# floe/backscrub

Hardware: AMD Instinct MI355X
Metric: composited frames/sec at 640×480 (batch), 1/2/4/8 MI355X + mask IoU vs CPU ref (higher is better)
Workload: dtype f32 (network) / u8 (image kernels)

## Files before the change

### backscrub_amd/csrc/bsx_api.hip

```cpp
#include "debug_switches.hpp"
#include <hip/hip_runtime.h>

#include <cmath>
#include <cstdarg>
#include <cstdio>
#include <cstdlib>
#include <cstring>
#include <map>
#include <memory>
#include <string>
#include <vector>

#include "../../include/bsx.h"
#include "gen_mid.hpp"
#include "gen_seg.hpp"
#include "kernels.hpp"
#include "roctx_ranges.hpp"
#include "rtc.hpp"
#include "plan.hpp"
#include "tflite_model.hpp"

using namespace bsx;

namespace {
// ... 191 lines not shown
  return "";
}

int model_type_from_name(const std::string& n) {
  if (n.find("body-pix") != n.npos) return BSX_MODEL_BODYPIX;
  if (n.find("deeplab") != n.npos) return BSX_MODEL_DEEPLAB;
  if (n.find("segm_") != n.npos) return BSX_MODEL_MEET;
  if (n.find("selfie") != n.npos) return BSX_MODEL_MLKIT;
  return BSX_MODEL_UNKNOWN;
}

int init_device_state(bsx_ctx* c) {
  BSX_HIP(c, hipStreamCreateWithFlags(&c->own_stream, hipStreamNonBlocking));
  const size_t N = (size_t)c->n_streams;
  BSX_HIP(c, hipMalloc(&c->d_arena, c->plan.arena_floats_per_stream * N * sizeof(float)));
  BSX_HIP(c, hipMalloc(&c->d_net_in, N * c->inW * c->inH * c->inC * sizeof(float)));
  BSX_HIP(c, hipMalloc(&c->d_net_in_u8, N * c->inW * c->inH * sizeof(uint32_t)));
  BSX_HIP(c, hipMalloc(&c->d_net_out, N * c->outW * c->outH * c->outC * sizeof(float)));
  BSX_HIP(c, hipMalloc(&c->d_weights, std::max<size_t>(c->plan.weights.size(), 4) * sizeof(float)));
  BSX_HIP(c, hipMemcpy(c->d_weights, c->plan.weights.data(), c->plan.weights.size() * sizeof(float), hipMemcpyHostToDevice));
  BSX_HIP(c, hipMalloc(&c->d_weights16, std::max<size_t>(c->plan.weights16.size(), 8) * sizeof(uint16_t)));
  BSX_HIP(c, hipMemcpy(c->d_weights16, c->plan.weights16.data(), c->plan.weights16.size() * sizeof(uint16_t), hipMemcpyHostToDevice));
  if (const char* m = getenv("BSX_F16_GEMM")) c->f16_terms = !strcmp(m, "off") ? 0 : (!strcmp(m, "fast") ? 1 : (!strcmp(m, "fast16") ? 17 : 3));
  c->use_program = !c->plan.program.empty() && BSX_DBG_ENV("BSX_NO_FRAME_PROGRAM") == nullptr &&
                   (c->plan.seg.on || c->plan.program_lds_tensors >= c->plan.program_global_tensors || BSX_DBG_ENV("BSX_FORCE_FRAME_PROGRAM") != nullptr);
  if (c->use_program) {
    BSX_HIP(c, hipMalloc(&c->d_program, c->plan.program.size() * sizeof(MicroOp)));
    BSX_HIP(c, hipMemcpy(c->d_program, c->plan.program.data(), c->plan.program.size() * sizeof(MicroOp), hipMemcpyHostToDevice));
    BSX_HIP(c, frame_program_prepare(c->plan.program_lds_floats));
    if (c->plan.seg.on) BSX_HIP(c, seg_prepare());
// ... 154 lines not shown
  if (logits || !c->seg_fn[2]) return launch_seg_tail(sp.tail, c->d_arena, pf, c->d_net_out, ofinal, c->d_weights, logits, n, s, c->act16);
  SegTail d = sp.tail; float* arena = c->d_arena; float* no = c->d_net_out; const float* w = c->d_weights; int nf = n;
  void* args[] = {&d, &arena, &pf, &no, &ofinal, &w, &nf};
  return seg_launch(c->seg_fn[2], d.tiles_y * d.tiles_x, n, d.lds_floats, s, args);
}

int run_infer(bsx_ctx* c, int n, hipStream_t s, bool logits = true, int slot = 0) {
  bsx_roctx::Range range("bsx:network");
  if (c->use_program && c->plan.seg.on) {
    const SegPlan& sp = c->plan.seg;
    const long pf = (long)c->plan.arena_floats_per_stream;
    BSX_HIP(c, seg_head(c, n, s));
    BSX_HIP(c, seg_k2(c, n, s));
    BSX_HIP(c, launch_program(c, n, s));
    BSX_HIP(c, seg_k3(c, n, s));
    if (sp.tail.pre_gate_off >= 0) BSX_HIP(c, launch_seg_gate(sp.tail.gate, c->d_arena, pf, c->d_weights, sp.tail.pre_gate_off, n, s));
    if (!logits) { const int frc = state_write_fence(c, s); if (frc) return frc; }
    BSX_HIP(c, seg_tail(c, c->d_ofinal + (size_t)slot * c->outW * c->outH, logits, n, s));
    return BSX_OK;
  }
  if (c->use_program) {
    BSX_HIP(c, launch_program(c, n, s));
    return BSX_OK;
  }
  const bool fused_tail = !logits && argmax_tail(c);
  const size_t ns = c->plan.steps.size() - (fused_tail ? 1 : 0);
  for (size_t i = 0; i < ns; i++)
    BSX_HIP(c, launch_step(c->plan.steps[i], c->plan, c->d_arena, c->d_net_in, c->d_net_out, c->d_weights, n, c->n_streams, s, c->d_weights16, c->f16_terms, c->in_u8 ? c->d_net_in_u8 : nullptr, c->norm_scale, c->norm_offset));
  if (fused_tail) {
    const Step& last = c->plan.steps.back();
    { const int frc = state_write_fence(c, s); if (frc) return frc; }
// ... 505 lines not shown
      if (!d_frames || !prep_yuyv_fusable(c->width, c->roi, c->tab_down.tab)) return BSX_EINVAL;
      return run_prep(c, d_frames, n, s, true, true);
    default: return BSX_EINVAL;
  }
}

int bsx_profile_batch(bsx_ctx* c, const uint8_t* d_frames, const uint8_t* d_bg, size_t bg_stride, uint8_t* d_out, int n, int iters,
                      bsx_launch_stat* out, int cap, void* stream) {
  if (!c || !d_frames || !d_bg || !d_out || !out || n <= 0 || n > c->n_streams || iters <= 0) return BSX_EINVAL;
  if (c->pend.active) { c->last_error = "error: a pipelined composite is pending (flush with bsx_step_batch_pipelined(ctx, NULL, ...) first)\n"; return BSX_EINVAL; }
  DeviceGuard guard(c->device);
  hipStream_t s = pick(c, stream);
  const bool seg = c->use_program && c->plan.seg.on;
  const bool fused_decode = infer_decodes(c);
  const bool atail = argmax_tail(c);
  const int n_net = c->use_program ? (seg ? (c->plan.seg.tail.pre_gate_off >= 0 ? 6 : 5) : 1) : (int)c->plan.steps.size();
  const bool fuse_tail = !c->onmask && !c->no_mask_blend_fusion &&
                         mask_blend_fusable(c->width, c->height, c->roi, d_bg, bg_stride, d_frames, d_out);
  const int L = 1 + n_net + (fused_decode ? 0 : 1) + (fuse_tail ? 1 : 2) + (fuse_tail ? 1 : 0);
  if (cap < L) return BSX_EINVAL;
  std::vector<hipEvent_t> ev((size_t)L + 1);
  for (auto& e : ev) BSX_HIP(c, hipEventCreate(&e));
  std::vector<double> sum(L, 0.0);
  const double N = n, px = (double)c->width * c->height;
  for (int it = 0; it < iters; it++) {
    int k = 0;
    BSX_HIP(c, hipEventRecord(ev[0], s));
#define BSX_TIMED(call)                                    \
    do {                                                   \
      BSX_HIP(c, (call));                                  \
      BSX_HIP(c, hipEventRecord(ev[k + 1], s));            \
      k++;                                                 \
    } while (0)
    BSX_TIMED(launch_prep_fused(d_frames, c->width, c->height, c->roi, c->in_u8 ? nullptr : c->tensor_ptr(c->plan.input), c->in_u8 ? c->d_net_in_u8 : nullptr, c->inW, c->inH, c->in_roi,
                                c->tab_down.tab, c->bilateral, n, s));
    const long pf = (long)c->plan.arena_floats_per_stream;
    if (seg) {
      const SegPlan& sp = c->plan.seg;
      BSX_TIMED(seg_head(c, n, s));
      BSX_TIMED(seg_k2(c, n, s));
      BSX_TIMED(launch_program(c, n, s));
      BSX_TIMED(seg_k3(c, n, s));
      if (sp.tail.pre_gate_off >= 0) BSX_TIMED(launch_seg_gate(sp.tail.gate, c->d_arena, pf, c->d_weights, sp.tail.pre_gate_off, n, s));
      BSX_TIMED(seg_tail(c, c->d_ofinal, !fused_decode, n, s));
    } else if (c->use_program)
      BSX_TIMED(launch_program(c, n, s));
    else {
      for (size_t si = 0; si + (atail ? 1 : 0) < c->plan.steps.size(); si++)
        BSX_TIMED(launch_step(c->plan.steps[si], c->plan, c->d_arena, c->d_net_in, c->d_net_out, c->d_weights, n, c->n_streams, s, c->d_weights16, c->f16_terms, c->in_u8 ? c->d_net_in_u8 : nullptr, c->norm_scale, c->norm_offset));
      if (atail) BSX_TIMED(launch_resize_argmax_iir(c->plan.steps.back(), c->d_arena + (size_t)c->plan.tensor_off[c->plan.steps.back().in0] * (size_t)c->n_streams,
                                                    c->d_ofinal, n, s, c->tail_generic));
    }
    if (!fused_decode) BSX_TIMED(launch_decode(c->model_type, c->tensor_ptr(c->plan.output), c->d_ofinal, c->outW * c->outH, c->outC, n, s));
    if (fuse_tail) {
      BSX_TIMED(launch_mask_blend(c->d_ofinal, c->outW, c->outH, c->in_roi, c->tab_up.tab, c->d_masks, c->width, c->height, c->roi, d_bg, bg_stride,
                                  d_frames, d_out, n, s));
      BSX_TIMED(launch_blend(d_bg, bg_stride, d_frames, c->d_masks, d_out, (size_t)c->width * c->height, n, s));
    } else {
// ... 13 lines not shown
  int j = 0;
  const double canvas = (double)c->inW * c->inH;
  const double touched = (double)std::min(c->roi.w, 2 * c->in_roi.w) * (double)std::min(c->roi.h, 2 * c->in_roi.h);
  put(j++, "prep", N * (3.0 * touched + (c->in_u8 ? 4.0 : 12.0) * canvas), 0);
  if (seg) {
    const std::vector<Step>& S = c->plan.steps;
    const int NS = (int)S.size();
    auto macs = [&](int a, int b) { double m = 0; for (int i = a; i <= b; i++) m += S[i].macs; return m; };
    const SegPlan& sp = c->plan.seg;
    const double eA = 16.0 * sp.head.H1 * sp.head.W1, eb0 = 16.0 * sp.head.H2 * sp.head.W2, ec0 = (double)sp.k2.dw.C * sp.k2.H3 * sp.k2.W3;
    const double elo2 = 16.0 * sp.k3.HL * sp.k3.WL, elo = 16.0 * sp.k3.H2 * sp.k3.W2;
    const double ein = (double)c->inW * c->inH * c->inC, eout = (double)c->outW * c->outH * c->outC;
    put(j++, "seg_head", N * ((c->in_u8 ? 4.0 * c->inW * c->inH : 4.0 * ein) + 4.0 * (eA + eb0)), N * 2.0 * macs(0, 2));
    put(j++, "seg_k2", N * 4.0 * (eb0 + eb0 + ec0), N * 2.0 * macs(3, 8));
    put(j++, "frame_program", N * 4.0 * (ec0 + elo2) + 4.0 * c->plan.weights.size(), N * 2.0 * macs(9, NS - 11));
    put(j++, "seg_k3", N * 4.0 * (eb0 + elo2 + elo), N * 2.0 * macs(NS - 10, NS - 8));
    if (sp.tail.pre_gate_off >= 0) put(j++, "seg_gate", N * 4.0 * (16.0 * (sp.tail.gate.part[0].n + sp.tail.gate.part[1].n) + 16.0), 0);
    put(j++, fused_decode ? "seg_tail+decode" : "seg_tail", N * (4.0 * (eA + elo) + (fused_decode ? 2.0 * c->outW * c->outH : 4.0 * eout)), N * 2.0 * macs(NS - 7, NS - 1));
  } else if (c->use_program) {
    double io = (double)c->inW * c->inH * c->inC + (double)c->outW * c->outH * c->outC;
    put(j++, "frame_program", N * io * 4.0 + 4.0 * c->plan.weights.size(), N * 2.0 * c->plan.macs_per_frame);
  } else
  for (const Step& st : c->plan.steps) {
    double in = (double)st.H * st.W * st.Cin, o = (double)st.OH * st.OW * st.Cout, b = 0;
    switch (st.kind) {
      case StepKind::Eltwise: b = in + o + (st.elt == kEltUnary ? 0 : (st.bcast1 ? st.Cin : in)) + (st.elt == kEltMulAdd ? in : 0); break;
      case StepKind::Concat: b = 2 * o; break;
      case StepKind::Gap: b = in + st.Cin; break;
      default: b = in + o + (st.residual >= 0 ? o : 0) + (st.in_scale >= 0 ? st.Cin : 0); break;
    }
    const bool is_tail = atail && &st == &c->plan.steps.back();
    const bool ir_on = c->d_weights16 && c->f16_terms > 0;
// ... 194 lines not shown
```

### backscrub_amd/csrc/gen_seg.cpp

```cpp
#include "gen_seg.hpp"

#include <cstdarg>
#include <cstdio>

namespace bsx {
namespace {

const char kSegSource[] =
#include "seg_rtc_src.inc"
    ;

}

std::string seg_constants_text(const SegPlan& sp, const char* pre) {
  std::string out;
  auto P = [&](const char* fmt, ...) {
    char buf[1024];
    va_list ap;
    va_start(ap, fmt);
    vsnprintf(buf, sizeof buf, fmt, ap);
    va_end(ap);
    out += buf;
  };
  auto conv = [&](const char* n, const SegConvW& c) { P("  t.%s.w_off = %lldll; t.%s.b_off = %lldll; t.%s.Cin = %d; t.%s.Cout = %d; t.%s.cout_pad = %d; t.%s.act = %d;\n", n, c.w_off, n, c.b_off, n, c.Cin, n, c.Cout, n, c.cout_pad, n, c.act); };
// ... 5 lines not shown
      P("  t.%s.fc[%d].w_off = %lldll; t.%s.fc[%d].b_off = %lldll; t.%s.fc[%d].Cin = %d; t.%s.fc[%d].Cout = %d; t.%s.fc[%d].act = %d;\n", n, i, g_.fc[i].w_off, n, i, g_.fc[i].b_off, n, i, g_.fc[i].Cin, n, i,
              g_.fc[i].Cout, n, i, g_.fc[i].act);
    }
  };
  const SegHead& H = sp.head; const SegK2& K2 = sp.k2; const SegK3& K3 = sp.k3; const SegTail& T = sp.tail;
  P("// segment descriptors of the loaded graph as constants (gen_seg.cpp: seg_constants_text)\nconstexpr SegHead %sHEAD = [] { SegHead t{};\n", pre);
  P("  t.H0 = %d; t.W0 = %d; t.H1 = %d; t.W1 = %d; t.H2 = %d; t.W2 = %d; t.stem_pt = %d; t.stem_pl = %d; t.dw_pt = %d; t.dw_pl = %d;\n", H.H0, H.W0, H.H1, H.W1, H.H2, H.W2, H.stem_pt, H.stem_pl, H.dw_pt, H.dw_pl);
  conv("stem", H.stem); conv("pw", H.pw); dw("dw", H.dw);
  P("  t.a_off = %lldll; t.b0_off = %lldll; t.part_a_off = %lldll; t.part_b0_off = %lldll; t.TR = %d; t.TC = %d; t.tiles_y = %d; t.tiles_x = %d; t.lds_floats = %d; t.rw = %d; t.m_ct = %uu;\n  return t; }();\n",
          H.a_off, H.b0_off, H.part_a_off, H.part_b0_off, H.TR, H.TC, H.tiles_y, H.tiles_x, H.lds_floats, H.rw, H.m_ct);
  P("constexpr SegK2 %sK2 = [] { SegK2 t{};\n  t.H2 = %d; t.W2 = %d; t.H3 = %d; t.W3 = %d; t.dw_pt = %d; t.dw_pl = %d;\n", pre, K2.H2, K2.W2, K2.H3, K2.W3, K2.dw_pt, K2.dw_pl);
  gate("gate", K2.gate); conv("pw_a", K2.pw_a); conv("pw_b", K2.pw_b); dw("dw", K2.dw);
  P("  t.b0_off = %lldll; t.B_off = %lldll; t.c0_off = %lldll; t.part_B_off = %lldll; t.TR = %d; t.TC = %d; t.tiles_y = %d; t.tiles_x = %d; t.lds_floats = %d; t.rw = %d; t.m_ct = %uu;\n  return t; }();\n",
          K2.b0_off, K2.B_off, K2.c0_off, K2.part_B_off, K2.TR, K2.TC, K2.tiles_y, K2.tiles_x, K2.lds_floats, K2.rw, K2.m_ct);
  P("constexpr SegK3 %sK3 = [] { SegK3 t{};\n  t.H2 = %d; t.W2 = %d; t.HL = %d; t.WL = %d; t.half_pixel = %d; t.align_corners = %d;\n", pre, K3.H2, K3.W2, K3.HL, K3.WL, K3.half_pixel, K3.align_corners);
  conv("pw1", K3.pw1); conv("pw2", K3.pw2); dw("dw", K3.dw);
  P("  t.skip_off = %lldll; t.lo2_off = %lldll; t.g_off = %lldll; t.lo_off = %lldll; t.part_lo_off = %lldll; t.TR = %d; t.TC = %d; t.tiles_y = %d; t.tiles_x = %d; t.lds_floats = %d; t.lo_floats = %d; t.hs = (float)%.9g; t.ws = (float)%.9g;\n  return t; }();\n",
          K3.skip_off, K3.lo2_off, K3.g_off, K3.lo_off, K3.part_lo_off, K3.TR, K3.TC, K3.tiles_y, K3.tiles_x, K3.lds_floats, K3.lo_floats, (double)K3.hs, (double)K3.ws);
  P("constexpr SegTail %sTAIL = [] { SegTail t{};\n  t.H1 = %d; t.W1 = %d; t.HL = %d; t.WL = %d; t.H0 = %d; t.W0 = %d; t.half_pixel = %d; t.align_corners = %d;\n", pre, T.H1, T.W1, T.HL, T.WL, T.H0, T.W0, T.half_pixel, T.align_corners);
  gate("gate", T.gate); conv("pw", T.pw); dw("dw", T.dw);
  P("  t.tc_w_off = %lldll; t.tc_b_off = %lldll; t.Co = %d; t.act3 = %d; t.model_type = %d; t.skip_off = %lldll; t.lo_off = %lldll; t.pre_gate_off = %lldll; t.TR = %d; t.TC = %d; t.tiles_y = %d; t.tiles_x = %d; "
             "t.lds_floats = %d; t.lo_floats = %d; t.hs = (float)%.9g; t.ws = (float)%.9g;\n  return t; }();\n",
          T.tc_w_off, T.tc_b_off, T.Co, T.act3, T.model_type, T.skip_off, T.lo_off, T.pre_gate_off, T.TR, T.TC, T.tiles_y, T.tiles_x, T.lds_floats, T.lo_floats, (double)T.hs, (double)T.ws);
  return out;
}

std::string generate_seg_source(const Plan& plan, bool h16, bool u8in, std::string* why) {
  auto fail = [&](const char* m) { if (why) *why = m; return std::string(); };
  if (!plan.seg.on) return fail("no segment kernels in this plan");
  const SegPlan& sp = plan.seg;
  const bool sig = sp.tail.act3 == kActSigmoid;
// ... 14 lines not shown
```

### backscrub_amd/csrc/kernels_seg.hip

```cpp
#ifndef __HIPCC_RTC__
#include <hip/hip_runtime.h>
#endif
#ifndef BSX_SEG_RTC
#include "debug_switches.hpp"

#include <algorithm>
#include <cstdlib>

#include "kernels.hpp"
#include "mfma_tile.hpp"
#include "segments.hpp"
#endif

#if defined(BSX_SEG_RTC)
#define BSX_SEG_D(T, NAME) constexpr T d = kSeg##NAME; (void)d_rt
#elif defined(BSX_SEG_PROBE)
#define BSX_SEG_D(T, NAME) constexpr T d = kProbe##NAME; (void)d_rt
#else
#define BSX_SEG_D(T, NAME) const T& d = d_rt
#endif

namespace bsx {
#ifdef BSX_SEG_RTC
namespace segrtc {
BSX_SEG_CONSTANTS
constexpr bool STEM_HSWISH = BSX_SEG_HS != 0, H16 = BSX_SEG_H16 != 0, U8IN = BSX_SEG_U8 != 0, LOGITS = false, SIGMOID = BSX_SEG_SIG != 0;
constexpr int CO = BSX_SEG_CO;
#else
namespace {
#endif
#ifdef BSX_SEG_PROBE
#include BSX_SEG_PROBE
#endif

extern __shared__ __attribute__((aligned(16))) float seg_smem[];

constexpr int kScrGate = 0;
constexpr int kScrRed = 96;
constexpr int kScrFloats = kSegScratchFloats;

__device__ __forceinline__ float4 ld4(const float* p) { return *reinterpret_cast<const float4*>(p); }
__device__ __forceinline__ void st4(float* p, float4 v) { *reinterpret_cast<float4*>(p) = v; }
// ... 42 lines not shown
__device__ __forceinline__ float4 acc_quad(const f4acc acc) { return make_float4(acc[0], acc[1], acc[2], acc[3]); }
__device__ __forceinline__ f4acc mma16(const float4 a, const float (&wr)[4]) {
  f4acc acc = {0.f, 0.f, 0.f, 0.f};
  acc = __builtin_amdgcn_mfma_f32_16x16x4f32(wr[0], a.x, acc, 0, 0, 0);
  acc = __builtin_amdgcn_mfma_f32_16x16x4f32(wr[1], a.y, acc, 0, 0, 0);
  acc = __builtin_amdgcn_mfma_f32_16x16x4f32(wr[2], a.z, acc, 0, 0, 0);
  acc = __builtin_amdgcn_mfma_f32_16x16x4f32(wr[3], a.w, acc, 0, 0, 0);
  return acc;
}
__device__ __forceinline__ void load_wtile(float (&wr)[4], const float* __restrict__ w, const SegConvW& c, int n0, int li, int g) {
#pragma unroll
  for (int r = 0; r < 4; r++) wr[r] = (w + c.w_off)[(unsigned)((4 * g + r) * c.cout_pad + n0 + li)];
}

constexpr int kGateStageFloats = kSegGateStageFloats;
__device__ __forceinline__ void seg_gate(const SegGate& gt, const float* __restrict__ fa, const float* __restrict__ w, float* scr, float* stage) {
  float* s_gate = scr + kScrGate;
  if (gt.timing_skip) { if (threadIdx.x < 16) s_gate[threadIdx.x] = 0.5f; __syncthreads(); return; }
  float* s_mean = scr + kScrGate + 16;
  float* s_hid = scr + kScrGate + 48;
  const int tid = threadIdx.x;
  const SegFc &f1 = gt.fc[0], &f2 = gt.fc[1];
  const int w1n = f1.Cin * f1.Cout, w2n = gt.n_fc == 2 ? f2.Cin * f2.Cout : 0;
  float* ps = stage;
  float* w1 = ps + 512;
  float* b1 = w1 + w1n;
  float* w2 = b1 + f1.Cout;
  float* b2 = w2 + w2n;
  {
    const int c = tid & 15, slice = tid >> 4;
    for (int k = 0; k < gt.n_parts; k++) {
      const float* src = fa + gt.part[k].off;
      float s = 0.f;
#pragma unroll 4
      for (int i = slice; i < gt.part[k].n; i += 16) s += src[(unsigned)(i * 16 + c)];
      ps[k * 256 + slice * 16 + c] = s;
    }
  }
  {
    const float* g1 = w + f1.w_off;
    const float* g2 = w + f2.w_off;
    for (int i = tid; i < w1n; i += kSegThreads) w1[i] = g1[(unsigned)i];
    for (int i = tid; i < w2n; i += kSegThreads) w2[i] = g2[(unsigned)i];
    if (tid < f1.Cout) b1[tid] = (w + f1.b_off)[(unsigned)tid];
    if (gt.n_fc == 2 && tid < f2.Cout) b2[tid] = (w + f2.b_off)[(unsigned)tid];
  }
  __syncthreads();
  const int Cm = gt.sum_parts ? 16 : 16 * gt.n_parts;
  if (tid < Cm) {
    float m = 0.f;
// ... 32 lines not shown
template <int MODE>
__device__ __forceinline__ void wave_reduce16(float4 v, float* s_red, int wave, int lane) {
  if (MODE == 0) {
    v.x += dpp_row_shr<1>(v.x); v.y += dpp_row_shr<1>(v.y); v.z += dpp_row_shr<1>(v.z); v.w += dpp_row_shr<1>(v.w);
    v.x += dpp_row_shr<2>(v.x); v.y += dpp_row_shr<2>(v.y); v.z += dpp_row_shr<2>(v.z); v.w += dpp_row_shr<2>(v.w);
    v.x += dpp_row_shr<4>(v.x); v.y += dpp_row_shr<4>(v.y); v.z += dpp_row_shr<4>(v.z); v.w += dpp_row_shr<4>(v.w);
    v.x += dpp_row_shr<8>(v.x); v.y += dpp_row_shr<8>(v.y); v.z += dpp_row_shr<8>(v.z); v.w += dpp_row_shr<8>(v.w);
    const int li = lane & 15;
    if (li >= 12) st4(s_red + (wave * 4 + (15 - li)) * 16 + 4 * (lane >> 4), li == 15 ? v : f4zero());
  } else {
    v.x += dpp_row_shr<4>(v.x); v.y += dpp_row_shr<4>(v.y); v.z += dpp_row_shr<4>(v.z); v.w += dpp_row_shr<4>(v.w);
    v.x += dpp_row_shr<8>(v.x); v.y += dpp_row_shr<8>(v.y); v.z += dpp_row_shr<8>(v.z); v.w += dpp_row_shr<8>(v.w);
    if ((lane & 12) == 12) st4(s_red + (wave * 4 + (lane >> 4)) * 16 + 4 * (lane & 3), v);
  }
}
__device__ __forceinline__ void store_partials(const float* s_red, float* dst ) {
  if (threadIdx.x < 16) {
    float s = 0.f;
#pragma unroll
    for (int j = 0; j < 16; j++) s += s_red[j * 16 + threadIdx.x];
    dst[threadIdx.x] = s;
  }
}

__device__ __forceinline__ void up_axis(int o, float scale, bool half_pixel, int in_size, int* lo, int* hi, float* frac) {
  const float v = half_pixel ? __fadd_rn(__fmul_rn((float)o + 0.5f, scale), -0.5f) : __fmul_rn((float)o, scale);
  const float fl = floorf(v);
  *lo = max((int)fl, 0);
  *hi = min((int)ceilf(v), in_size - 1);
  *frac = v - (float)*lo;
}
__device__ __forceinline__ float up_scale(int in, int out, bool align) { return (align && out > 1) ? (float)(in - 1) / (float)(out - 1) : (float)in / (float)out; }

__device__ __forceinline__ float quad_reduce_scatter(float p0, float p1, float p2, float p3, int quad) {
  const bool b0 = quad & 1, b1 = quad & 2;
  const float klo = (b0 ? p1 : p0) + dpp_quad(b0 ? p0 : p1, 1);
// ... 357 lines not shown
    float4 a;
    a.x = fmaf(sk.x, gv.x, fmaf(td.x, w11, fmaf(tc.x, w01, fmaf(tb.x, w10, ta.x * w00))));
    a.y = fmaf(sk.y, gv.y, fmaf(td.y, w11, fmaf(tc.y, w01, fmaf(tb.y, w10, ta.y * w00))));
    a.z = fmaf(sk.z, gv.z, fmaf(td.z, w11, fmaf(tc.z, w01, fmaf(tb.z, w10, ta.z * w00))));
    a.w = fmaf(sk.w, gv.w, fmaf(td.w, w11, fmaf(tc.w, w01, fmaf(tb.w, w10, ta.w * w00))));
    const f4acc acc = mma16(a, wr);
    float4 v = acc_quad(acc);
    v = (ecol_in && row_in) ? clamp4(f4add(v, bias), cl) : f4zero();
    if (xe < ZC) st4(z_t + zy * 256 + col_a(xe, g), v);
  }
}

#ifdef BSX_SEG_RTC
extern "C" __global__ __launch_bounds__(kSegThreads) void bsx_seg_k3(
#else
template <bool H16>
__global__ __launch_bounds__(kSegThreads) void seg_k3_k(
#endif
    const SegK3 d_rt, float* __restrict__ arena, long per_frame, const float* __restrict__ w, int n_frames) {
  BSX_SEG_D(SegK3, K3);
  unsigned f_, t_;
  xcd_frame_tile((unsigned)(d.tiles_y * d.tiles_x), (unsigned)n_frames, &f_, &t_);
  const int f = (int)f_, ty = (int)t_ / d.tiles_x, tx = (int)t_ - ty * d.tiles_x;
  const int r0 = ty * d.TR, c0 = tx * d.TC, ZH = d.TR + 2, ZC = d.TC + 2;
  float* fa = arena + (size_t)f * (size_t)per_frame;
  float* z_t = seg_smem + kScrFloats;
  float* l_t = z_t + ZH * 256;
  float* lo_out = fa + d.lo_off;
  const int tid = threadIdx.x, lane = tid & 63, wave = wave_uniform(tid >> 6), li = lane & 15, g = lane >> 4, cq4 = 4 * g;
  const GatedPre pre = gated_prefetch<H16>(fa + d.skip_off, fa + d.lo2_off, d.H2, d.W2, d.HL, d.WL, d.half_pixel != 0, d.hs, d.ws, r0, c0, ZH, ZC, l_t);
  if (tid < 16) seg_smem[kScrGate + tid] = fa[d.g_off + tid];
// ... 14 lines not shown
  const int xe = li;
  for (int py = wave; py < d.TR && r0 + py < d.H2; py += 4) {
    const f4v zc = ldv(z_t + (py + 1) * 256 + coz[1]);
    const float4 dv = clamp4(tof4(dw3x3(z_t, 256, py, coz, wd) + bias_d), cl_dw);
    const f4acc acc = mma16(f4add(dv, tof4(zc)), wr);
    float4 v = acc_quad(acc);
    if (xe < d.TC && c0 + xe < d.W2) {
      v = clamp4(f4add(v, bias2), cl_2);
      stg4<H16>(lo_out, (unsigned)(((r0 + py) * d.W2 + c0 + xe) * 16 + cq4), v);
      sum = f4add(sum, v);
    }
  }
  float* s_red = seg_smem + kScrRed;
  wave_reduce16<0>(sum, s_red, wave, lane);
  __syncthreads();
  store_partials(s_red, fa + d.part_lo_off + (long)t_ * 16);
}

#ifdef BSX_SEG_RTC
extern "C" __global__ __launch_bounds__(kSegThreads) __attribute__((amdgpu_waves_per_eu(5, 5))) void bsx_seg_tail(
#else
template <int CO, bool LOGITS, bool SIGMOID, bool H16>
__global__ __launch_bounds__(kSegThreads) __attribute__((amdgpu_waves_per_eu(5, 5))) void seg_tail_k(
#endif
    const SegTail d_rt, float* __restrict__ arena, long per_frame, float* __restrict__ net_out,
                                                          uint8_t* __restrict__ ofinal, const float* __restrict__ w, int n_frames) {
  BSX_SEG_D(SegTail, TAIL);
  unsigned f_, t_;
  xcd_frame_tile((unsigned)(d.tiles_y * d.tiles_x), (unsigned)n_frames, &f_, &t_);
  const int f = (int)f_, ty = (int)t_ / d.tiles_x, tx = (int)t_ - ty * d.tiles_x;
  const int r0 = ty * d.TR, c0 = tx * d.TC, ZH = d.TR + 2, ZC = d.TC + 2;
// ... 75 lines not shown
template <class K>
hipError_t allow_lds(K kernel, int lds_bytes) {
  return hipFuncSetAttribute(reinterpret_cast<const void*>(kernel), hipFuncAttributeMaxDynamicSharedMemorySize, lds_bytes);
}
#endif

}

#ifndef BSX_SEG_RTC
hipError_t seg_prepare() {
  const int full = 160 * 1024;
  hipError_t e = hipSuccess;
  auto one = [&](auto k) { if (e == hipSuccess) e = allow_lds(k, full); };
  one(seg_head_k<true, false, false>); one(seg_head_k<false, false, false>); one(seg_head_k<true, true, false>); one(seg_head_k<false, true, false>);
  one(seg_head_k<true, false, true>); one(seg_head_k<false, false, true>); one(seg_head_k<true, true, true>); one(seg_head_k<false, true, true>);
  one(seg_k2_k<false>); one(seg_k2_k<true>); one(seg_k3_k<false>); one(seg_k3_k<true>);
  one(seg_tail_k<1, false, true, false>); one(seg_tail_k<1, true, true, false>); one(seg_tail_k<1, false, false, false>); one(seg_tail_k<1, true, false, false>);
  one(seg_tail_k<2, false, false, false>); one(seg_tail_k<2, true, false, false>);
  one(seg_tail_k<1, false, true, true>); one(seg_tail_k<1, true, true, true>); one(seg_tail_k<1, false, false, true>); one(seg_tail_k<1, true, false, true>);
  one(seg_tail_k<2, false, false, true>); one(seg_tail_k<2, true, false, true>);
  return e;
}

static int xcd_frames(int n) { static const bool on = !(BSX_DBG_ENV("BSX_XCD_TILES") && atoi(BSX_DBG_ENV("BSX_XCD_TILES")) == 0); return on ? n : 0; }

hipError_t launch_seg_head(const SegHead& d, float* arena, long per_frame, const void* net_in, const float* weights, int n, hipStream_t s, bool h16, bool u8, float in_scale,
                           float in_offset) {
  const dim3 grid((unsigned)(d.tiles_y * d.tiles_x) * (unsigned)n);
  const size_t lds = (size_t)d.lds_floats * sizeof(float);
  const bool hs = d.stem.act == kActHswish;
  const float* in = static_cast<const float*>(net_in);
  if (u8 && 2 * (2 * d.TC + 1) + 1 > 64) return hipErrorInvalidValue;
#define BSX_HEAD(HS, H, U) seg_head_k<HS, H, U><<<grid, kSegThreads, lds, s>>>(d, arena, per_frame, in, weights, in_scale, in_offset, xcd_frames(n))
  if (hs) { if (h16) { if (u8) BSX_HEAD(true, true, true); else BSX_HEAD(true, true, false); } else { if (u8) BSX_HEAD(true, false, true); else BSX_HEAD(true, false, false); } }
  else { if (h16) { if (u8) BSX_HEAD(false, true, true); else BSX_HEAD(false, true, false); } else { if (u8) BSX_HEAD(false, false, true); else BSX_HEAD(false, false, false); } }
#undef BSX_HEAD
  return hipGetLastError();
}
hipError_t launch_seg_k2(const SegK2& d, float* arena, long per_frame, const float* weights, int n, hipStream_t s, bool h16) {
  const dim3 grid((unsigned)(d.tiles_y * d.tiles_x) * (unsigned)n);
  if (h16) seg_k2_k<true><<<grid, kSegThreads, (size_t)d.lds_floats * sizeof(float), s>>>(d, arena, per_frame, weights, xcd_frames(n));
  else seg_k2_k<false><<<grid, kSegThreads, (size_t)d.lds_floats * sizeof(float), s>>>(d, arena, per_frame, weights, xcd_frames(n));
  return hipGetLastError();
}
hipError_t launch_seg_k3(const SegK3& d, float* arena, long per_frame, const float* weights, int n, hipStream_t s, bool h16) {
  const dim3 grid((unsigned)(d.tiles_y * d.tiles_x) * (unsigned)n);
  if (h16) seg_k3_k<true><<<grid, kSegThreads, (size_t)d.lds_floats * sizeof(float), s>>>(d, arena, per_frame, weights, xcd_frames(n));
  else seg_k3_k<false><<<grid, kSegThreads, (size_t)d.lds_floats * sizeof(float), s>>>(d, arena, per_frame, weights, xcd_frames(n));
  return hipGetLastError();
}
template <bool H16>
static hipError_t launch_seg_tail_t(const SegTail& d, float* arena, long per_frame, float* net_out, uint8_t* ofinal, const float* weights, bool logits, int n, hipStream_t s) {
  const dim3 grid((unsigned)(d.tiles_y * d.tiles_x) * (unsigned)n);
  static const int wgs_cap = BSX_DBG_ENV("BSX_SEG_TAIL_WGS") ? atoi(BSX_DBG_ENV("BSX_SEG_TAIL_WGS")) : 0;
  size_t lds = (size_t)d.lds_floats * sizeof(float);
  if (wgs_cap > 0) lds = std::max(lds, (size_t)(160 * 1024 / (wgs_cap + 1) + 256));
  const bool sig = d.act3 == kActSigmoid;
  if (d.Co == 2 && !sig) {
    if (logits) seg_tail_k<2, true, false, H16><<<grid, kSegThreads, lds, s>>>(d, arena, per_frame, net_out, ofinal, weights, xcd_frames(n));
    else seg_tail_k<2, false, false, H16><<<grid, kSegThreads, lds, s>>>(d, arena, per_frame, net_out, ofinal, weights, xcd_frames(n));
  } else if (d.Co == 1 && sig) {
    if (logits) seg_tail_k<1, true, true, H16><<<grid, kSegThreads, lds, s>>>(d, arena, per_frame, net_out, ofinal, weights, xcd_frames(n));
    else seg_tail_k<1, false, true, H16><<<grid, kSegThreads, lds, s>>>(d, arena, per_frame, net_out, ofinal, weights, xcd_frames(n));
// ... 20 lines not shown
```

### backscrub_amd/csrc/plan.cpp

```cpp
#include "debug_switches.hpp"
#include "plan.hpp"
#include "gen_seg.hpp"
#include "gen_mid.hpp"

#include <algorithm>
#include <cmath>
#include <cstdio>
#include <cstdlib>
#include <cstring>
#include <map>

namespace bsx {
namespace {

void conv_geometry(int in, int k, int s, int d, bool same, int* out, int* pad) {
  int eff = (k - 1) * d + 1;
  *out = same ? (in + s - 1) / s : (in + s - eff) / s;
  int total = (*out - 1) * s + eff - in;
  *pad = total > 0 ? total / 2 : 0;
}

uint16_t f32_to_f16_rn(float f) {
  uint32_t x; memcpy(&x, &f, 4);
  const uint32_t sign = (x >> 16) & 0x8000u;
// ... 600 lines not shown
  tl.pw = conv_w(tpw); tl.dw = dw_w(tdw); tl.tc_w_off = (long long)ttc.w_off; tl.tc_b_off = (long long)ttc.b_off; tl.Co = ttc.Cout; tl.act3 = ttc.act;
  split(tl.H1, tgt[6], &tl.TR, &tl.tiles_y); split(tl.W1, tgt[7], &tl.TC, &tl.tiles_x);
  tl.hs = seg_up_scale(tl.HL, tl.H1, tl.align_corners != 0); tl.ws = seg_up_scale(tl.WL, tl.W1, tl.align_corners != 0);
  if (!BSX_DBG_ENV("BSX_SEG_LO_WORST")) tl.lo_floats = seg_lo_window_floats(tl.H1, tl.W1, tl.HL, tl.WL, tl.half_pixel != 0, tl.align_corners != 0, tl.TR, tl.TC, tl.tiles_y, tl.tiles_x);
  tl.lds_floats = seg_tail_lds_floats(tl);
  if (tl.TC > 14 || tl.TR > 18) return seg_fail(33);
  const int lds_cap = 160 * 256;
  if (h.lds_floats > lds_cap || k2.lds_floats > lds_cap || k3.lds_floats > lds_cap || tl.lds_floats > lds_cap) return seg_fail(24);
  if (ttc.OH != 2 * tpw.OH || ttc.OW != 2 * tpw.OW || h.H2 != k3.H2 || h.W2 != k3.W2) return seg_fail(25);
  if (h.tiles_y * h.tiles_x > 1024 || k2.tiles_y * k2.tiles_x > 1024 || k3.tiles_y * k3.tiles_x > 1024) return seg_fail(26);

  const int pA = synth("partials(A)", h.tiles_y * h.tiles_x, 16), pb0 = synth("partials(b0)", h.tiles_y * h.tiles_x, 16);
  const int pB = synth("partials(B)", k2.tiles_y * k2.tiles_x, 16), plo = synth("partials(lo)", k3.tiles_y * k3.tiles_x, 16);
  const int pgt = BSX_DBG_ENV("BSX_SEG_NO_GATE_KERNEL") ? -1 : synth("gate(tail)", 1, 16);
  if (pgt >= 0) plan->tensor_off[pgt] = reserve(16);
  for (int t : {A, b0, B, c0, lo2, lo, kf2.out, pA, pb0, pB, plo}) plan->tensor_off[t] = reserve(g.tensors[t].elems());
  for (int t : {hpw.out, g1.out, f1a.out, f1b.out, pwb.out, up2, kg.out, kf1.out, kp1.out, kd.out, up, tg.out, tf1.out, tf2.out, tpw.out, tdw.out})
    if (t != g.output) plan->tensor_off[t] = -1;
  plan->arena_floats_per_stream = top;

  h.a_off = plan->tensor_off[A]; h.b0_off = plan->tensor_off[b0]; h.part_a_off = plan->tensor_off[pA]; h.part_b0_off = plan->tensor_off[pb0];
  k2.b0_off = plan->tensor_off[b0]; k2.B_off = plan->tensor_off[B]; k2.c0_off = plan->tensor_off[c0]; k2.part_B_off = plan->tensor_off[pB];
  k2.gate.n_parts = 1; k2.gate.n_fc = 2; k2.gate.sum_parts = 0;
  k2.gate.part[0].off = plan->tensor_off[pb0]; k2.gate.part[0].n = h.tiles_y * h.tiles_x; k2.gate.part[0].C = 16; k2.gate.part[0].hw = (float)(h.H2 * h.W2);
  k2.gate.fc[0] = fc_w(f1a); k2.gate.fc[1] = fc_w(f1b);
  k3.skip_off = plan->tensor_off[B]; k3.lo2_off = plan->tensor_off[lo2]; k3.g_off = plan->tensor_off[kf2.out]; k3.lo_off = plan->tensor_off[lo];
  k3.part_lo_off = plan->tensor_off[plo];
  tl.skip_off = plan->tensor_off[A]; tl.lo_off = plan->tensor_off[lo];
  tl.gate.n_parts = 2; tl.gate.n_fc = 2; tl.gate.sum_parts = tg.gap_sum ? 1 : 0;
  tl.gate.part[0].off = plan->tensor_off[pA]; tl.gate.part[0].n = h.tiles_y * h.tiles_x; tl.gate.part[0].C = 16; tl.gate.part[0].hw = (float)(h.H1 * h.W1);
  tl.gate.part[1].off = plan->tensor_off[plo]; tl.gate.part[1].n = k3.tiles_y * k3.tiles_x; tl.gate.part[1].C = 16; tl.gate.part[1].hw = (float)(k3.H2 * k3.W2);
  tl.gate.fc[0] = fc_w(tf1); tl.gate.fc[1] = fc_w(tf2);
  if (BSX_DBG_ENV("BSX_SEG_GATE_SKIP")) k2.gate.timing_skip = tl.gate.timing_skip = 1;
  if (const char* e = BSX_DBG_ENV("BSX_SEG_SKIP")) sscanf(e, "%d,%d,%d,%d", &h.dbg_skip, &k2.dbg_skip, &k3.dbg_skip, &tl.dbg_skip);
  tl.pre_gate_off = pgt >= 0 ? plan->tensor_off[pgt] : -1;
  if (tl.gate.fc[0].Cin != (tl.gate.sum_parts ? 16 : 32) || k2.gate.fc[0].Cin != 16) return seg_fail(27);

  std::vector<Step> mid(S.begin() + 9, S.begin() + (NS - 14));
  Step gate = kg;
  gate.concat_in = {B, lo2};
  gate.in0 = B;
  gate.label += "*";
  mid.push_back(gate); mid.push_back(kf1); mid.push_back(kf2);
  std::map<int, int> part_n, part_hw;
  part_n[B] = k2.tiles_y * k2.tiles_x; part_hw[B] = k2.H2 * k2.W2;
  const long B_real = plan->tensor_off[B];
  plan->tensor_off[B] = plan->tensor_off[pB];
  build_frame_program(g, plan, mid, {c0, B, lo2, kf2.out}, part_n, part_hw);
  plan->tensor_off[B] = B_real;
  if (plan->program.empty()) return seg_fail(28);
// ... 558 lines not shown
```

### backscrub_amd/csrc/segments.hpp

```cpp
#pragma once
#ifndef BSX_SEG_RTC
#include <algorithm>
#include <cmath>
#include <cstdint>
#endif

namespace bsx {

struct SegConvW { long long w_off = 0, b_off = 0; int Cin = 0, Cout = 0, cout_pad = 0, act = 0; };
struct SegDwW { long long w_off = 0, b_off = 0; int C = 0, act = 0; };
struct SegFc { long long w_off = 0, b_off = 0; int Cin = 0, Cout = 0, act = 0; };
struct SegPart { long long off = 0; int n = 0, C = 0; float hw = 1.f; };
struct SegGate {
  int n_parts = 0, sum_parts = 0, n_fc = 0;
  int timing_skip = 0;
  SegPart part[2];
  SegFc fc[2];
};

constexpr int kSegThreads = 256;
constexpr int kSegMaxC = 16;

struct SegHead {
  int H0 = 0, W0 = 0, H1 = 0, W1 = 0, H2 = 0, W2 = 0;
// ... 21 lines not shown
  int rw = 0;
  unsigned m_ct = 0;
};

struct SegK3 {
  int H2 = 0, W2 = 0, HL = 0, WL = 0;
  int half_pixel = 0, align_corners = 0;
  SegConvW pw1, pw2;
  SegDwW dw;
  long long skip_off = 0, lo2_off = 0, g_off = 0, lo_off = 0, part_lo_off = 0;
  int TR = 0, TC = 0, tiles_y = 0, tiles_x = 0;
  int lds_floats = 0;
  int lo_floats = 0;
  float hs = 0.f, ws = 0.f;
  int dbg_skip = 0;
};

struct SegTail {
  int H1 = 0, W1 = 0, HL = 0, WL = 0, H0 = 0, W0 = 0;
  int half_pixel = 0, align_corners = 0;
  SegGate gate;
  SegConvW pw;
  SegDwW dw;
  long long tc_w_off = 0, tc_b_off = 0;
  int Co = 0, act3 = 0, model_type = 0;
  long long skip_off = 0, lo_off = 0;
  long long pre_gate_off = -1;
  int TR = 0, TC = 0, tiles_y = 0, tiles_x = 0;
  int lds_floats = 0;
  int lo_floats = 0;
// ... 55 lines not shown
```

Before: 729,600.

## Fold tail gate computation into seg_k3 via last-block arrival counter

Removes the separate seg_gate kernel launch by having the last-arriving tile block of seg_k3 compute the tail gate from the partial sums. Each block stores its partials with agent-scope atomic stores and increments an arena counter, and the block that arrives last reads all partials atomically and writes the gate vector. This saves one launch and one dependency gap per frame batch. In exchange the kernel carries more template variants, the arena needs a one-time memset so the counter starts at zero, and correctness relies on memory ordering that uses relaxed atomics plus an s_waitcnt.

```diff
diff --git a/backscrub_amd/csrc/bsx_api.hip b/backscrub_amd/csrc/bsx_api.hip
--- a/backscrub_amd/csrc/bsx_api.hip
+++ b/backscrub_amd/csrc/bsx_api.hip
@@ -229,6 +229,8 @@
   BSX_HIP(c, hipStreamCreateWithFlags(&c->own_stream, hipStreamNonBlocking));
   const size_t N = (size_t)c->n_streams;
   BSX_HIP(c, hipMalloc(&c->d_arena, c->plan.arena_floats_per_stream * N * sizeof(float)));
+  if (c->plan.seg.on && c->plan.seg.k3.gate_fold)
+    BSX_HIP(c, hipMemset(c->d_arena, 0, c->plan.arena_floats_per_stream * N * sizeof(float)));
   BSX_HIP(c, hipMalloc(&c->d_net_in, N * c->inW * c->inH * c->inC * sizeof(float)));
   BSX_HIP(c, hipMalloc(&c->d_net_in_u8, N * c->inW * c->inH * sizeof(uint32_t)));
   BSX_HIP(c, hipMalloc(&c->d_net_out, N * c->outW * c->outH * c->outC * sizeof(float)));
@@ -413,7 +415,7 @@
     BSX_HIP(c, seg_k2(c, n, s));
     BSX_HIP(c, launch_program(c, n, s));
     BSX_HIP(c, seg_k3(c, n, s));
-    if (sp.tail.pre_gate_off >= 0) BSX_HIP(c, launch_seg_gate(sp.tail.gate, c->d_arena, pf, c->d_weights, sp.tail.pre_gate_off, n, s));
+    if (sp.tail.pre_gate_off >= 0 && !sp.k3.gate_fold) BSX_HIP(c, launch_seg_gate(sp.tail.gate, c->d_arena, pf, c->d_weights, sp.tail.pre_gate_off, n, s));
     if (!logits) { const int frc = state_write_fence(c, s); if (frc) return frc; }
     BSX_HIP(c, seg_tail(c, c->d_ofinal + (size_t)slot * c->outW * c->outH, logits, n, s));
     return BSX_OK;
@@ -949,7 +951,7 @@
   const bool seg = c->use_program && c->plan.seg.on;
   const bool fused_decode = infer_decodes(c);
   const bool atail = argmax_tail(c);
-  const int n_net = c->use_program ? (seg ? (c->plan.seg.tail.pre_gate_off >= 0 ? 6 : 5) : 1) : (int)c->plan.steps.size();
+  const int n_net = c->use_program ? (seg ? (c->plan.seg.tail.pre_gate_off >= 0 && !c->plan.seg.k3.gate_fold ? 6 : 5) : 1) : (int)c->plan.steps.size();
   const bool fuse_tail = !c->onmask && !c->no_mask_blend_fusion &&
                          mask_blend_fusable(c->width, c->height, c->roi, d_bg, bg_stride, d_frames, d_out);
   const int L = 1 + n_net + (fused_decode ? 0 : 1) + (fuse_tail ? 1 : 2) + (fuse_tail ? 1 : 0);
@@ -976,7 +978,7 @@
       BSX_TIMED(seg_k2(c, n, s));
       BSX_TIMED(launch_program(c, n, s));
       BSX_TIMED(seg_k3(c, n, s));
-      if (sp.tail.pre_gate_off >= 0) BSX_TIMED(launch_seg_gate(sp.tail.gate, c->d_arena, pf, c->d_weights, sp.tail.pre_gate_off, n, s));
+      if (sp.tail.pre_gate_off >= 0 && !sp.k3.gate_fold) BSX_TIMED(launch_seg_gate(sp.tail.gate, c->d_arena, pf, c->d_weights, sp.tail.pre_gate_off, n, s));
       BSX_TIMED(seg_tail(c, c->d_ofinal, !fused_decode, n, s));
     } else if (c->use_program)
       BSX_TIMED(launch_program(c, n, s));
@@ -1020,8 +1022,9 @@
     put(j++, "seg_head", N * ((c->in_u8 ? 4.0 * c->inW * c->inH : 4.0 * ein) + 4.0 * (eA + eb0)), N * 2.0 * macs(0, 2));
     put(j++, "seg_k2", N * 4.0 * (eb0 + eb0 + ec0), N * 2.0 * macs(3, 8));
     put(j++, "frame_program", N * 4.0 * (ec0 + elo2) + 4.0 * c->plan.weights.size(), N * 2.0 * macs(9, NS - 11));
-    put(j++, "seg_k3", N * 4.0 * (eb0 + elo2 + elo), N * 2.0 * macs(NS - 10, NS - 8));
-    if (sp.tail.pre_gate_off >= 0) put(j++, "seg_gate", N * 4.0 * (16.0 * (sp.tail.gate.part[0].n + sp.tail.gate.part[1].n) + 16.0), 0);
+    const double k3_gate = sp.k3.gate_fold ? 4.0 * (16.0 * (sp.tail.gate.part[0].n + sp.tail.gate.part[1].n) + 16.0) : 0.0;
+    put(j++, "seg_k3", N * (4.0 * (eb0 + elo2 + elo) + k3_gate), N * 2.0 * macs(NS - 10, NS - 8));
+    if (sp.tail.pre_gate_off >= 0 && !sp.k3.gate_fold) put(j++, "seg_gate", N * 4.0 * (16.0 * (sp.tail.gate.part[0].n + sp.tail.gate.part[1].n) + 16.0), 0);
     put(j++, fused_decode ? "seg_tail+decode" : "seg_tail", N * (4.0 * (eA + elo) + (fused_decode ? 2.0 * c->outW * c->outH : 4.0 * eout)), N * 2.0 * macs(NS - 7, NS - 1));
   } else if (c->use_program) {
     double io = (double)c->inW * c->inH * c->inC + (double)c->outW * c->outH * c->outC;
diff --git a/backscrub_amd/csrc/gen_seg.cpp b/backscrub_amd/csrc/gen_seg.cpp
--- a/backscrub_amd/csrc/gen_seg.cpp
+++ b/backscrub_amd/csrc/gen_seg.cpp
@@ -43,7 +43,8 @@
   P("  t.b0_off = %lldll; t.B_off = %lldll; t.c0_off = %lldll; t.part_B_off = %lldll; t.TR = %d; t.TC = %d; t.tiles_y = %d; t.tiles_x = %d; t.lds_floats = %d; t.rw = %d; t.m_ct = %uu;\n  return t; }();\n",
           K2.b0_off, K2.B_off, K2.c0_off, K2.part_B_off, K2.TR, K2.TC, K2.tiles_y, K2.tiles_x, K2.lds_floats, K2.rw, K2.m_ct);
   P("constexpr SegK3 %sK3 = [] { SegK3 t{};\n  t.H2 = %d; t.W2 = %d; t.HL = %d; t.WL = %d; t.half_pixel = %d; t.align_corners = %d;\n", pre, K3.H2, K3.W2, K3.HL, K3.WL, K3.half_pixel, K3.align_corners);
-  conv("pw1", K3.pw1); conv("pw2", K3.pw2); dw("dw", K3.dw);
+  conv("pw1", K3.pw1); conv("pw2", K3.pw2); dw("dw", K3.dw); gate("tgate", K3.tgate);
+  P("  t.gate_fold = %d; t.tgate_off = %lldll; t.count_off = %lldll;\n", K3.gate_fold, K3.tgate_off, K3.count_off);
   P("  t.skip_off = %lldll; t.lo2_off = %lldll; t.g_off = %lldll; t.lo_off = %lldll; t.part_lo_off = %lldll; t.TR = %d; t.TC = %d; t.tiles_y = %d; t.tiles_x = %d; t.lds_floats = %d; t.lo_floats = %d; t.hs = (float)%.9g; t.ws = (float)%.9g;\n  return t; }();\n",
           K3.skip_off, K3.lo2_off, K3.g_off, K3.lo_off, K3.part_lo_off, K3.TR, K3.TC, K3.tiles_y, K3.tiles_x, K3.lds_floats, K3.lo_floats, (double)K3.hs, (double)K3.ws);
   P("constexpr SegTail %sTAIL = [] { SegTail t{};\n  t.H1 = %d; t.W1 = %d; t.HL = %d; t.WL = %d; t.H0 = %d; t.W0 = %d; t.half_pixel = %d; t.align_corners = %d;\n", pre, T.H1, T.W1, T.HL, T.WL, T.H0, T.W0, T.half_pixel, T.align_corners);
diff --git a/backscrub_amd/csrc/kernels_seg.hip b/backscrub_amd/csrc/kernels_seg.hip
--- a/backscrub_amd/csrc/kernels_seg.hip
+++ b/backscrub_amd/csrc/kernels_seg.hip
@@ -26,6 +26,7 @@
 BSX_SEG_CONSTANTS
 constexpr bool STEM_HSWISH = BSX_SEG_HS != 0, H16 = BSX_SEG_H16 != 0, U8IN = BSX_SEG_U8 != 0, LOGITS = false, SIGMOID = BSX_SEG_SIG != 0;
 constexpr int CO = BSX_SEG_CO;
+constexpr bool K3_GATE = kSegK3.gate_fold != 0;
 #else
 namespace {
 #endif
@@ -98,6 +99,9 @@
 }
 
 constexpr int kGateStageFloats = kSegGateStageFloats;
+template <bool SC1>
+__device__ __forceinline__ float ld_part(const float* p) { return SC1 ? __hip_atomic_load(p, __ATOMIC_RELAXED, __HIP_MEMORY_SCOPE_AGENT) : *p; }
+template <bool SC1 = false>
 __device__ __forceinline__ void seg_gate(const SegGate& gt, const float* __restrict__ fa, const float* __restrict__ w, float* scr, float* stage) {
   float* s_gate = scr + kScrGate;
   if (gt.timing_skip) { if (threadIdx.x < 16) s_gate[threadIdx.x] = 0.5f; __syncthreads(); return; }
@@ -117,7 +121,7 @@
       const float* src = fa + gt.part[k].off;
       float s = 0.f;
 #pragma unroll 4
-      for (int i = slice; i < gt.part[k].n; i += 16) s += src[(unsigned)(i * 16 + c)];
+      for (int i = slice; i < gt.part[k].n; i += 16) s += ld_part<SC1>(src + (unsigned)(i * 16 + c));
       ps[k * 256 + slice * 16 + c] = s;
     }
   }
@@ -180,12 +184,14 @@
     if ((lane & 12) == 12) st4(s_red + (wave * 4 + (lane >> 4)) * 16 + 4 * (lane & 3), v);
   }
 }
+template <bool SC1 = false>
 __device__ __forceinline__ void store_partials(const float* s_red, float* dst ) {
   if (threadIdx.x < 16) {
     float s = 0.f;
 #pragma unroll
     for (int j = 0; j < 16; j++) s += s_red[j * 16 + threadIdx.x];
-    dst[threadIdx.x] = s;
+    if (SC1) __hip_atomic_store(dst + threadIdx.x, s, __ATOMIC_RELAXED, __HIP_MEMORY_SCOPE_AGENT);
+    else dst[threadIdx.x] = s;
   }
 }
 
@@ -573,7 +579,7 @@
 #ifdef BSX_SEG_RTC
 extern "C" __global__ __launch_bounds__(kSegThreads) void bsx_seg_k3(
 #else
-template <bool H16>
+template <bool H16, bool K3_GATE>
 __global__ __launch_bounds__(kSegThreads) void seg_k3_k(
 #endif
     const SegK3 d_rt, float* __restrict__ arena, long per_frame, const float* __restrict__ w, int n_frames) {
@@ -618,7 +624,23 @@
   float* s_red = seg_smem + kScrRed;
   wave_reduce16<0>(sum, s_red, wave, lane);
   __syncthreads();
-  store_partials(s_red, fa + d.part_lo_off + (long)t_ * 16);
+  store_partials<K3_GATE>(s_red, fa + d.part_lo_off + (long)t_ * 16);
+  if (K3_GATE) {
+    unsigned* cnt = reinterpret_cast<unsigned*>(fa + d.count_off);
+    float* s_last = seg_smem + kScrRed - 4;
+    if (tid == 0) {
+      asm volatile("s_waitcnt vmcnt(0)" ::: "memory");
+      const unsigned old = __hip_atomic_fetch_add(cnt, 1u, __ATOMIC_RELAXED, __HIP_MEMORY_SCOPE_AGENT);
+      const bool last = old == (unsigned)(d.tiles_y * d.tiles_x - 1);
+      if (last) __hip_atomic_store(cnt, 0u, __ATOMIC_RELAXED, __HIP_MEMORY_SCOPE_AGENT);
+      s_last[0] = last ? 1.f : 0.f;
+    }
+    __syncthreads();
+    if (s_last[0] != 0.f) {
+      seg_gate<true>(d.tgate, fa, w, seg_smem, z_t);
+      if (tid < 16) fa[d.tgate_off + tid] = seg_smem[kScrGate + tid];
+    }
+  }
 }
 
 #ifdef BSX_SEG_RTC
@@ -724,7 +746,7 @@
   auto one = [&](auto k) { if (e == hipSuccess) e = allow_lds(k, full); };
   one(seg_head_k<true, false, false>); one(seg_head_k<false, false, false>); one(seg_head_k<true, true, false>); one(seg_head_k<false, true, false>);
   one(seg_head_k<true, false, true>); one(seg_head_k<false, false, true>); one(seg_head_k<true, true, true>); one(seg_head_k<false, true, true>);
-  one(seg_k2_k<false>); one(seg_k2_k<true>); one(seg_k3_k<false>); one(seg_k3_k<true>);
+  one(seg_k2_k<false>); one(seg_k2_k<true>); one(seg_k3_k<false, false>); one(seg_k3_k<true, false>); one(seg_k3_k<false, true>); one(seg_k3_k<true, true>);
   one(seg_tail_k<1, false, true, false>); one(seg_tail_k<1, true, true, false>); one(seg_tail_k<1, false, false, false>); one(seg_tail_k<1, true, false, false>);
   one(seg_tail_k<2, false, false, false>); one(seg_tail_k<2, true, false, false>);
   one(seg_tail_k<1, false, true, true>); one(seg_tail_k<1, true, true, true>); one(seg_tail_k<1, false, false, true>); one(seg_tail_k<1, true, false, true>);
@@ -755,8 +777,14 @@
 }
 hipError_t launch_seg_k3(const SegK3& d, float* arena, long per_frame, const float* weights, int n, hipStream_t s, bool h16) {
   const dim3 grid((unsigned)(d.tiles_y * d.tiles_x) * (unsigned)n);
-  if (h16) seg_k3_k<true><<<grid, kSegThreads, (size_t)d.lds_floats * sizeof(float), s>>>(d, arena, per_frame, weights, xcd_frames(n));
-  else seg_k3_k<false><<<grid, kSegThreads, (size_t)d.lds_floats * sizeof(float), s>>>(d, arena, per_frame, weights, xcd_frames(n));
+  const size_t lds = (size_t)d.lds_floats * sizeof(float);
+  if (d.gate_fold) {
+    if (h16) seg_k3_k<true, true><<<grid, kSegThreads, lds, s>>>(d, arena, per_frame, weights, xcd_frames(n));
+    else seg_k3_k<false, true><<<grid, kSegThreads, lds, s>>>(d, arena, per_frame, weights, xcd_frames(n));
+  } else {
+    if (h16) seg_k3_k<true, false><<<grid, kSegThreads, lds, s>>>(d, arena, per_frame, weights, xcd_frames(n));
+    else seg_k3_k<false, false><<<grid, kSegThreads, lds, s>>>(d, arena, per_frame, weights, xcd_frames(n));
+  }
   return hipGetLastError();
 }
 template <bool H16>
diff --git a/backscrub_amd/csrc/plan.cpp b/backscrub_amd/csrc/plan.cpp
--- a/backscrub_amd/csrc/plan.cpp
+++ b/backscrub_amd/csrc/plan.cpp
@@ -638,6 +638,9 @@
   const int pB = synth("partials(B)", k2.tiles_y * k2.tiles_x, 16), plo = synth("partials(lo)", k3.tiles_y * k3.tiles_x, 16);
   const int pgt = BSX_DBG_ENV("BSX_SEG_NO_GATE_KERNEL") ? -1 : synth("gate(tail)", 1, 16);
   if (pgt >= 0) plan->tensor_off[pgt] = reserve(16);
+  k3.gate_fold = pgt >= 0 && !BSX_DBG_ENV("BSX_SEG_GATE_KERNEL") && k3.lds_floats - kSegScratchFloats >= kSegGateStageFloats;
+  const int pcnt = k3.gate_fold ? synth("arrivals(k3)", 1, 16) : -1;
+  if (pcnt >= 0) plan->tensor_off[pcnt] = reserve(16);
   for (int t : {A, b0, B, c0, lo2, lo, kf2.out, pA, pb0, pB, plo}) plan->tensor_off[t] = reserve(g.tensors[t].elems());
   for (int t : {hpw.out, g1.out, f1a.out, f1b.out, pwb.out, up2, kg.out, kf1.out, kp1.out, kd.out, up, tg.out, tf1.out, tf2.out, tpw.out, tdw.out})
     if (t != g.output) plan->tensor_off[t] = -1;
@@ -658,6 +661,7 @@
   if (BSX_DBG_ENV("BSX_SEG_GATE_SKIP")) k2.gate.timing_skip = tl.gate.timing_skip = 1;
   if (const char* e = BSX_DBG_ENV("BSX_SEG_SKIP")) sscanf(e, "%d,%d,%d,%d", &h.dbg_skip, &k2.dbg_skip, &k3.dbg_skip, &tl.dbg_skip);
   tl.pre_gate_off = pgt >= 0 ? plan->tensor_off[pgt] : -1;
+  if (k3.gate_fold) { k3.tgate = tl.gate; k3.tgate_off = tl.pre_gate_off; k3.count_off = plan->tensor_off[pcnt]; }
   if (tl.gate.fc[0].Cin != (tl.gate.sum_parts ? 16 : 32) || k2.gate.fc[0].Cin != 16) return seg_fail(27);
 
   std::vector<Step> mid(S.begin() + 9, S.begin() + (NS - 14));
diff --git a/backscrub_amd/csrc/segments.hpp b/backscrub_amd/csrc/segments.hpp
--- a/backscrub_amd/csrc/segments.hpp
+++ b/backscrub_amd/csrc/segments.hpp
@@ -59,6 +59,9 @@
   int lo_floats = 0;
   float hs = 0.f, ws = 0.f;
   int dbg_skip = 0;
+  int gate_fold = 0;
+  SegGate tgate;
+  long long tgate_off = -1, count_off = -1;
 };
 
 struct SegTail {
```

Result: no change. 729,300 (median of 6 runs) (-0.0%).
